# zju3dv/LoG

Hardware: AMD Instinct MI355X
Metric: Gaussians/sec fwd+bwd @1080p (higher is better)
Workload: dtype f32; 1 GPU; 30M random Gaussians (seed 0, opacity 0.999), 1920x1080, 8 orbit views/GPU, fwd+bwd; north_star / configs[3] per GPU; gaussians=30000000, width=1920, height=1080, views_per_gpu=8, streams_per_gpu=1, parallelism=single GPU, 1 view(s) in flight per GPU (HIP streams)

## Files before the change

### log_amd/csrc/blend.hip

```cpp
#include "common.hpp"
#define LR_LANDED(q0, q1, c, i)                                                                                  \
  asm volatile("" : "+v"((q0).x), "+v"((q0).y), "+v"((q0).z), "+v"((q0).w), "+v"((q1).x), "+v"((q1).y), "+v"((q1).z), \
               "+v"((q1).w), "+v"(c), "+v"(i))
#define LR_OCC_ATTR(n) __attribute__((amdgpu_waves_per_eu(n)))
#ifdef LR_OCC_BWD_ROWS_WAVES
#define LR_OCC_BWD_ROWS LR_OCC_ATTR(LR_OCC_BWD_ROWS_WAVES)
#else
#define LR_OCC_BWD_ROWS
#endif
#ifndef LR_OCC_FWD_ROWS_WAVES
#define LR_OCC_FWD_ROWS_WAVES 5
#endif
#define LR_OCC_FWD_ROWS LR_OCC_ATTR(LR_OCC_FWD_ROWS_WAVES)
#ifdef LR_OCC_BWD_WAVES
#define LR_OCC_BWD LR_OCC_ATTR(LR_OCC_BWD_WAVES)
#else
#define LR_OCC_BWD
#endif
#ifdef LR_OCC_FWD_WAVES
#define LR_OCC_FWD LR_OCC_ATTR(LR_OCC_FWD_WAVES)
#else
#define LR_OCC_FWD
#endif


LR_DEV uint32_t lr_tile_of_block(uint32_t b, uint32_t tiles, int gx, int gy, int mode,
                                 const uint32_t* __restrict__ state) {
  if (mode == 3) return b < tiles ? state[lr_order_off(tiles) + b] : 0xffffffffu;
  if (mode == 1) {
    uint32_t nper = (tiles + 7u) >> 3;
    uint32_t t = (b & 7u) * nper + (b >> 3);
    return t < tiles ? t : 0xffffffffu;
  }
  if (mode == 2) {
    uint32_t nsbx = ((uint32_t)gx + 3u) >> 2, nsby = ((uint32_t)gy + 3u) >> 2;
    uint32_t r = b >> 3, sb = (r >> 4) * 8u + (b & 7u), local = r & 15u;
    if (sb >= nsbx * nsby) return 0xffffffffu;
    uint32_t tx = (sb % nsbx) * 4u + (local & 3u), ty = (sb / nsbx) * 4u + (local >> 2);
    if (tx >= (uint32_t)gx || ty >= (uint32_t)gy) return 0xffffffffu;
    return ty * (uint32_t)gx + tx;
  }
  return b < tiles ? b : 0xffffffffu;
}
static inline __host__ __device__ uint32_t lr_blend_grid(uint32_t tiles, int gx, int gy, int mode) {
  if (mode == 1) return ((tiles + 7u) / 8u) * 8u;
  if (mode == 2) {
    uint32_t nsb = (((uint32_t)gx + 3u) >> 2) * (((uint32_t)gy + 3u) >> 2);
    return ((nsb + 7u) / 8u) * 8u * 16u;
  }
  return tiles;
}

LR_DEV bool lr_support_hits(const float4 g0, const float2 g1, float x0, float x1, float y0, float y1) {
  const float A = g0.z, B = g0.w, C = g1.x, op = g1.y;
  const float det = A * C - B * B;
  const float tau = lr_fma(__logf(255.f * op), 1.01f, 0.01f);
  if (!(op >= 1.0f / 512.0f)) return !(op < 1.0f / 512.0f);
  const float inv = 1.f / det;
  const float ex2 = 2.f * tau * C * inv, ey2 = 2.f * tau * A * inv;
  const float mag = (fabsf(A) + fabsf(B) + fabsf(C)) * (ex2 + ey2);
  const bool safe = (det > 0.f) && (ex2 >= 0.f) && (ey2 >= 0.f) && (mag * 1.0e-6f < 0.005f * tau) && (mag < 1.0e30f);
  if (!safe) return true;
  const float ex = sqrtf(ex2) + 0.01f, ey = sqrtf(ey2) + 0.01f;
  if (!((g0.x + ex >= x0) && (g0.x - ex <= x1) && (g0.y + ey >= y0) && (g0.y - ey <= y1))) return false;
  const float dx0 = (x0 - 0.01f) - g0.x, dx1 = (x1 + 0.01f) - g0.x;
  const float dy0 = (y0 - 0.01f) - g0.y, dy1 = (y1 + 0.01f) - g0.y;
  if (dx0 <= 0.f && dx1 >= 0.f && dy0 <= 0.f && dy1 >= 0.f) return true;
  const float iA = 1.f / A, iC = 1.f / C;
  float best = 3.0e38f;
#pragma unroll
  for (int e = 0; e < 2; e++) {
    const float dx = e ? dx1 : dx0;
    const float dy = fminf(dy1, fmaxf(dy0, -B * dx * iC));
    best = fminf(best, 0.5f * (A * dx * dx + C * dy * dy) + B * dx * dy);
    const float ey_ = e ? dy1 : dy0;
    const float ex_ = fminf(dx1, fmaxf(dx0, -B * ey_ * iA));
    best = fminf(best, 0.5f * (A * ex_ * ex_ + C * ey_ * ey_) + B * ex_ * ey_);
  }
  return !(best > tau);
}

LR_DEV bool lr_lazy_range(const uint32_t* sorted, uint32_t tiles, int lazy, uint32_t tile, int wave, uint32_t beg,
                          uint32_t& end, uint32_t& first, bool& clamped) {
  first = 0u;
  clamped = false;
  if (!lazy) return true;
  if (end - beg <= LR_LONG_LIST) return lazy == 1;
  const uint32_t ordered = sorted[tile] & ~63u;
  if (lazy == 1) {
    if (ordered < end - beg) { end = beg + ordered; clamped = true; }
    return true;
  }
  if (!((sorted[tiles + tile] >> wave) & 1u)) return false;
  first = ordered;
  return true;
}
template <bool EXTRAS>
LR_DEV void lr_lazy_park(const LrView& v, size_t pix, bool done, float T, float C0, float C1, float C2, int last, int wid,
                         float wmax, float* image, float* final_T, int* n_contrib, int* pid, float* pwp) {
  const size_t plane = (size_t)v.W * v.H;
  final_T[pix] = done ? -T : T;
  n_contrib[pix] = last;
  image[pix] = C0; image[plane + pix] = C1; image[2 * plane + pix] = C2;
  if (EXTRAS) { pid[pix] = wid; pwp[pix] = wmax; }
}
template <bool EXTRAS>
LR_DEV void lr_lazy_resume(const LrView& v, size_t pix, bool& done, float& T, float& C0, float& C1, float& C2, int& last,
                           int& wid, float& wmax, const float* image, const float* final_T, const int* n_contrib,
                           const int* pid, const float* pwp) {
  const size_t plane = (size_t)v.W * v.H;
  const float t = final_T[pix];
  done = t < 0.f;
  T = fabsf(t);
  last = n_contrib[pix];
  C0 = image[pix]; C1 = image[plane + pix]; C2 = image[2 * plane + pix];
  if (EXTRAS) { wid = pid[pix]; wmax = pwp[pix]; }
}

#define LR_MBUF_CHUNKS 64u
#define LR_MASK_FORM_ROWS 1u
#define LR_MASK_FORM_QUAD 2u
LR_DEV size_t lr_mask_slot(uint32_t list_begin, uint32_t tile) { return (size_t)(list_begin >> 6) + tile; }
LR_DEV uint64_t lr_mask_before(uint64_t m, int hi, int limit) {
  const int sh = hi - limit;
  return sh <= 0 ? m : (sh >= 64 ? 0ull : (m & (~0ull << sh)));
}

template <bool EXTRAS>
LR_DEV void lr_fwd_commit_chunk(uint32_t* wmx, int lane, uint32_t id_prev, float* __restrict__ pw, float4* __restrict__ zero_rows) {
  if (!EXTRAS) return;
  __builtin_amdgcn_fence(__ATOMIC_RELEASE, "wavefront");
  __builtin_amdgcn_wave_barrier();
  __builtin_amdgcn_fence(__ATOMIC_ACQUIRE, "wavefront");
  const uint32_t m = (id_prev != 0xffffffffu) ? wmx[lane] : 0u;
  if (m != 0u) atomicMax(reinterpret_cast<unsigned int*>(pw) + id_prev, m);
  if (zero_rows) {
#pragma unroll
    for (int k = 0; k < 4; k++) {
      const int e = 16 * k + (lane >> 2);
      const uint32_t me = (uint32_t)__shfl((int)m, e), ide = (uint32_t)__shfl((int)id_prev, e);
      if (me != 0u) zero_rows[4 * (size_t)ide + (lane & 3)] = float4{0.f, 0.f, 0.f, 0.f};
    }
  }
  wmx[lane] = 0u;
  __builtin_amdgcn_fence(__ATOMIC_RELEASE, "wavefront");
  __builtin_amdgcn_wave_barrier();
}

template <bool EXTRAS>
__global__ void __launch_bounds__(256) LR_OCC_FWD
lr_blend_fwd_kernel(LrView v, const float4* __restrict__ geom, const uint32_t* __restrict__ state,
                    uint32_t tiles, const uint32_t* __restrict__ plist, uint32_t capacity,
                    float* __restrict__ image, float* __restrict__ final_T, int* __restrict__ n_contrib,
                    int* __restrict__ pid, float* __restrict__ pwp, float* __restrict__ pw,
                    float4* __restrict__ zero_conic, int xcd_mode, int cull, uint32_t* __restrict__ lazy_state, int lazy,
                    uint64_t* __restrict__ masks, uint32_t* __restrict__ hdr_w) {
  if (lr_bail(state, capacity)) return;
  if (lazy == 2 && !lazy_state[LR_HDR_OPEN]) return;
  if (masks && blockIdx.x == 0 && threadIdx.x == 0) hdr_w[LR_HDR_MASKS] = LR_MASK_FORM_QUAD;
  const uint32_t tile = lr_tile_of_block(blockIdx.x, tiles, v.gx, v.gy, xcd_mode, state);
  if (tile >= tiles) return;
// ... 174 lines not shown
  const int px = qx0 + (lane & 7), py = qy0 + (lane >> 3);
  const float pxf = (float)px, pyf = (float)py;
  const float bx0 = (float)qx0, bx1 = (float)(qx0 + 7), by0 = (float)qy0, by1 = (float)(qy0 + 7);
  const bool in = (px < v.W) && (py < v.H);
  const size_t plane = (size_t)v.W * v.H;
  const size_t pix = in ? (size_t)py * v.W + px : 0;
  const float sx = 0.5f * (float)v.W, sy = 0.5f * (float)v.H;
  const float Tf = in ? final_T[pix] : 0.f;
  const int lastc = in ? n_contrib[pix] : 0;
  const float dp0 = in ? dL_dimage[pix] : 0.f;
  const float dp1 = in ? dL_dimage[plane + pix] : 0.f;
  const float dp2 = in ? dL_dimage[2 * plane + pix] : 0.f;
  const float bgdot = lr_fma(v.bg[0], dp0, lr_fma(v.bg[1], dp1, v.bg[2] * dp2));
  float T = Tf, acc0 = 0.f, acc1 = 0.f, acc2 = 0.f;
  int maxc = lastc;
#pragma unroll
  for (int off = 32; off > 0; off >>= 1) maxc = max(maxc, __shfl_xor(maxc, off));
  maxc = lr_readlane_i(maxc, 0);

  const int row = lane >> 4;
  float* const base0 = acc_rows + ((row < 3) ? 6 + row : 5);
  float* const base1 = acc_rows + ((lane == 1) ? 4 : row);
  const bool lead = (lane & 15) == 0;

  const int top = use_masks ? ((maxc + 63) & ~63) : maxc;
  const uint32_t nchunks = ((uint32_t)top + 63u) >> 6;
  auto load_id = [&](uint32_t c) -> uint32_t {
    const int pos = top - 1 - (int)(c * 64u) - lane;
    return (c < nchunks && pos >= 0 && pos < maxc) ? plist[beg + (uint32_t)pos] : 0xffffffffu;
  };
  const uint64_t* const mbase = use_masks ? masks + 4 * lr_mask_slot(beg, tile) + __builtin_amdgcn_readfirstlane(quad) : nullptr;
  auto load_mask = [&](uint32_t c) -> uint64_t {
    return (use_masks && c < nchunks) ? mbase[4 * (size_t)(((uint32_t)top >> 6) - 1u - c)] : 0ull;
  };
  uint32_t id_n = load_id(0), id_nn = load_id(1);
  uint64_t mk_n = load_mask(0), mk_nn = load_mask(1);
  float4 g0_n = {0.f, 0.f, 0.f, 0.f};
  float2 g1_n = {0.f, 0.f};
  if (!use_masks && id_n != 0xffffffffu) { g0_n = geom[LR_REC_QUADS * (size_t)id_n]; g1_n = *reinterpret_cast<const float2*>(geom + LR_REC_QUADS * (size_t)id_n + 1); }

  for (uint32_t ch = 0; ch < nchunks; ch++) {
    const int hi = top - (int)(ch * 64u);
    const uint32_t id = id_n;
    const float4 g0 = g0_n;
    const float2 g1 = g1_n;
    const uint64_t mk = mk_n;
    id_n = id_nn;
    id_nn = load_id(ch + 2);
    mk_n = mk_nn;
    mk_nn = load_mask(ch + 2);
    uint64_t todo;
    if (use_masks) {
      todo = lr_mask_before(__builtin_bitreverse64(mk), hi, maxc);
    } else {
      if (id_n != 0xffffffffu) { g0_n = geom[LR_REC_QUADS * (size_t)id_n]; g1_n = *reinterpret_cast<const float2*>(geom + LR_REC_QUADS * (size_t)id_n + 1); }
      const bool rel = (id != 0xffffffffu) && (cull ? lr_support_hits(g0, g1, bx0, bx1, by0, by1) : true);
      todo = __ballot(rel);
    }
    while (todo) {
      const int j0 = __builtin_ctzll(todo);
      todo &= todo - 1;
      const bool has1 = todo != 0;
      const int j1 = has1 ? __builtin_ctzll(todo) : j0;
      todo &= todo - 1;
      const int gid0 = lr_readlane_i((int)id, j0), gid1 = lr_readlane_i((int)id, j1);
      const float4* __restrict__ rr0 = geom + LR_REC_QUADS * (size_t)(uint32_t)gid0;
      const float4* __restrict__ rr1 = geom + LR_REC_QUADS * (size_t)(uint32_t)gid1;
      const float4 q00 = rr0[0], q01 = rr0[1], q10 = rr1[0], q11 = rr1[1];
      const float cbl0 = reinterpret_cast<const float*>(rr0)[8], cbl1 = reinterpret_cast<const float*>(rr1)[8];
      asm volatile("" : : "s"(q01.z), "s"(q01.w), "s"(cbl0), "s"(q11.z), "s"(q11.w), "s"(cbl1));
      const float op0 = q01.y, op1 = q11.y;
      const lr_f2 dx2 = lr_f2{q00.x, q10.x} - pxf, dy2 = lr_f2{q00.y, q10.y} - pyf;
      const lr_f2 hdx2 = dx2 * -0.5f, hdy2 = dy2 * -0.5f;
      const lr_f2 bdx = lr_f2{q00.w, q10.w} * dx2;
      const lr_f2 pw2 = lr_fma2(lr_f2{q00.z, q10.z} * dx2, hdx2,
                                lr_fma2(lr_f2{q01.x, q11.x} * dy2, hdy2, lr_f2{-bdx.x, -bdx.y} * dy2));
      const lr_f2 G2 = lr_exp2(pw2);
      const lr_f2 al2 = lr_f2{op0, op1} * G2;
      const float power0 = pw2.x, power1 = pw2.y, G0 = G2.x, G1 = G2.y;
      const float alpha0 = fminf(0.99f, al2.x), alpha1 = fminf(0.99f, al2.y);
      const int k0 = hi - 1 - j0, k1 = hi - 1 - j1;
      const bool hit0 = (k0 < lastc) & !(power0 > 0.f) & !(alpha0 < 1.0f / 255.0f);
      const bool hit1 = has1 & (k1 < lastc) & !(power1 > 0.f) & !(alpha1 < 1.0f / 255.0f);
      const lr_f2 alpha = {hit0 ? alpha0 : 0.f, hit1 ? alpha1 : 0.f};
      const bool any0 = __builtin_amdgcn_ballot_w64(alpha.x > 0.f) != 0, any1 = __builtin_amdgcn_ballot_w64(alpha.y > 0.f) != 0;
      if (!(any0 | any1)) continue;
      const lr_f2 G = {hit0 ? G0 : 0.f, hit1 ? G1 : 0.f};
      const lr_f2 om = 1.f - alpha;
      lr_f2 rc = {__builtin_amdgcn_rcpf(om.x), __builtin_amdgcn_rcpf(om.y)};
      rc = lr_fma2(lr_fma2(-om, rc, lr_f2{1.f, 1.f}), rc, rc);
      const float Ta = T * rc.x, Tb = Ta * rc.y;
      const lr_f2 T2 = {Ta, Tb};
      T = Tb;
      const lr_f2 w = alpha * T2;
      const lr_f2 cr = {q01.z, q11.z}, cg = {q01.w, q11.w}, cbl = {cbl0, cbl1};
      const float a0r = lr_fma(alpha.x, cr.x, om.x * acc0), a0g = lr_fma(alpha.x, cg.x, om.x * acc1),
                  a0b = lr_fma(alpha.x, cbl.x, om.x * acc2);
      lr_f2 dL_dalpha = lr_fma2(cr - lr_f2{acc0, a0r}, lr_f2{dp0, dp0},
                                lr_fma2(cg - lr_f2{acc1, a0g}, lr_f2{dp1, dp1}, (cbl - lr_f2{acc2, a0b}) * dp2));
      dL_dalpha = lr_fma2(dL_dalpha, T2, -(Tf * rc) * bgdot);
      acc0 = lr_fma(alpha.y, cr.y, om.y * a0r);
      acc1 = lr_fma(alpha.y, cg.y, om.y * a0g);
      acc2 = lr_fma(alpha.y, cbl.y, om.y * a0b);
      const lr_f2 Ar = {q00.z, q10.z}, Br = {q00.w, q10.w}, Cr = {q01.x, q11.x};
      const lr_f2 dL_dG = lr_f2{op0, op1} * dL_dalpha;
      const lr_f2 gdx = G * dx2, gdy = G * dy2;
      const lr_f2 dG_ddx = lr_fma2(-Ar, gdx, -(Br * gdy));
      const lr_f2 dG_ddy = lr_fma2(-Cr, gdy, -(Br * gdx));
      lr_f2 s2[9];
      s2[0] = w * dp0; s2[2] = w * dp1; s2[1] = w * dp2; s2[3] = G * dL_dalpha;
      s2[4] = dL_dG * dG_ddx * sx; s2[6] = dL_dG * dG_ddy * sy;
      s2[5] = -0.5f * gdx * dx2 * dL_dG; s2[7] = -gdx * dy2 * dL_dG;
      s2[8] = -0.5f * gdy * dy2 * dL_dG;
#pragma unroll
      for (int e = 0; e < 2; e++) {
        if (!(e ? any1 : any0)) continue;
        const int gid = e ? gid1 : gid0;
        float sv[9];
#pragma unroll
        for (int m = 0; m < 9; m++) sv[m] = e ? s2[m].y : s2[m].x;
        float r0, r1, r2;
        lr_reduce9(sv, r0, r1, r2);
        if (lead) atomicAdd(base0 + (size_t)gid * LOGRAST_BWD_ROW_FLOATS, r0);
        if (lead || lane == 1) atomicAdd(base1 + (size_t)gid * LOGRAST_BWD_ROW_FLOATS, lane == 1 ? r2 : r1);
      }
    }
  }
}

#define LR_RB_SLOT 3
template <int CTRL>
LR_DEV float lr_dpp_perm(float x) {
  return __int_as_float(__builtin_amdgcn_update_dpp(0, __float_as_int(x), CTRL, 0xf, 0xf, true));
}
template <int BANKS>
LR_DEV float lr_bank_select(float keep, float take) {
  return __int_as_float(__builtin_amdgcn_update_dpp(__float_as_int(keep), __float_as_int(take), 0xE4, 0xf, BANKS, false));
}
LR_DEV float lr_row_pair8(float a, float b) {
  return lr_bank_select<0xc>(a + lr_dpp_perm<0x140>(a), b + lr_dpp_perm<0x140>(b));
}
LR_DEV float lr_row_pair4(float p, float q) {
  return lr_bank_select<0xa>(p + lr_dpp_perm<0x141>(p), q + lr_dpp_perm<0x141>(q));
}
LR_DEV float lr_quad_total(float x) {
  x = x + lr_dpp_perm<0xB1>(x);
  return x + lr_dpp_perm<0x4E>(x);
}

LR_DEV void lr_atomic_add_noret(float* p, float x) {
  asm volatile("global_atomic_add_f32 %0, %1, off" : : "v"(p), "v"(x) : "memory");
}

LR_DEV uint32_t lr_take_bit(uint64_t& m) {
  const uint32_t j = min((uint32_t)(__ffsll((long long)m) - 1), 64u);
  m &= m - 1ull;
  return j;
}
LR_DEV uint64_t lr_row_mask(int row, uint64_t m0, uint64_t m1, uint64_t m2, uint64_t m3) {
  return row == 0 ? m0 : (row == 1 ? m1 : (row == 2 ? m2 : m3));
}

template <bool MASKS>
__global__ void __launch_bounds__(256) LR_OCC_BWD_ROWS
lr_blend_bwd_rows_kernel(LrView v, const float4* __restrict__ geom, const uint32_t* __restrict__ state,
                         uint32_t tiles, const uint32_t* __restrict__ plist, uint32_t capacity,
                         const float* __restrict__ final_T, const int* __restrict__ n_contrib,
                         const float* __restrict__ dL_dimage, float* __restrict__ acc_rows,
                         int xcd_mode, int cull, int block_test, const uint64_t* __restrict__ masks LR_ABLATE_PARAM) {
  __shared__ float4 lr_stage[4][65 * LR_RB_SLOT];
  if (lr_bail(state, capacity)) return;
  const uint32_t tile = lr_tile_of_block(blockIdx.x, tiles, v.gx, v.gy, xcd_mode, state);
  if (tile >= tiles) return;
  const uint32_t* offsets = state + lr_offsets_off(tiles);
  const uint32_t beg = offsets[tile];
  const int lane = threadIdx.x & 63, wq = threadIdx.x >> 6;
  constexpr bool use_masks = MASKS;
  const int row = lane >> 4, li = lane & 15;
  const int tx = tile % (uint32_t)v.gx, ty = tile / (uint32_t)v.gx;
  const int qx0 = tx * 16 + (wq & 1) * 8, qy0 = ty * 16 + (wq >> 1) * 8;
  const int px = qx0 + (row & 1) * 4 + (li & 3), py = qy0 + (row >> 1) * 4 + (li >> 2);
  const float pxf = (float)px, pyf = (float)py;
  const bool in = (px < v.W) && (py < v.H);
  const size_t plane = (size_t)v.W * v.H;
  const size_t pix = in ? (size_t)py * v.W + px : 0;
  const float sx = 0.5f * (float)v.W, sy = 0.5f * (float)v.H;
  const float Tf = in ? final_T[pix] : 0.f;
  const int lastc = in ? n_contrib[pix] : 0;
  const float dp0 = in ? dL_dimage[pix] : 0.f;
  const float dp1 = in ? dL_dimage[plane + pix] : 0.f;
  const float dp2 = in ? dL_dimage[2 * plane + pix] : 0.f;
  const float bgdot = lr_fma(v.bg[0], dp0, lr_fma(v.bg[1], dp1, v.bg[2] * dp2));
  float T = Tf, acc0 = 0.f, acc1 = 0.f, acc2 = 0.f;
  int rmax = lastc;
#pragma unroll
  for (int off = 8; off > 0; off >>= 1) rmax = max(rmax, __shfl_xor(rmax, off));
  const int rm0 = lr_readlane_i(rmax, 0), rm1 = lr_readlane_i(rmax, 16), rm2 = lr_readlane_i(rmax, 32),
            rm3 = lr_readlane_i(rmax, 48);
  const int maxc = max(max(rm0, rm1), max(rm2, rm3));
  if (maxc == 0) return;

  float* const sf = reinterpret_cast<float*>(lr_stage[wq]);
#define LR_SF(f, j) sf[(f) * 65 + (j)]
  const uint32_t sf_lds = (uint32_t)(uintptr_t)(__attribute__((address_space(3))) float*)sf;
  if (lane < 10) LR_SF(lane, 64) = lane == 9 ? __uint_as_float(0xffffffffu) : 0.f;

  const int qd = li >> 2, sel = li & 3;
  const int slot = sel == 0 ? (qd == 0 ? 6 : (qd == 1 ? 8 : (qd == 2 ? 7 : 5)))
                            : (sel == 1 ? (qd == 0 ? 0 : (qd == 1 ? 2 : (qd == 2 ? 1 : 3))) : 4);
  const bool on_a = sel < 2 || li == 2, on_b = sel < 2 || li == 10;
  float* const dst = acc_rows + slot;

  const float bx[2] = {(float)qx0, (float)(qx0 + 4)}, by[2] = {(float)qy0, (float)(qy0 + 4)};

  const int top = use_masks ? ((maxc + 63) & ~63) : maxc;
  const uint32_t nchunks = ((uint32_t)top + 63u) >> 6;
  auto load_id = [&](uint32_t c) -> uint32_t {
    const int pos = top - 1 - (int)(c * 64u) - lane;
    const bool ok = c < nchunks && pos >= 0 && pos < maxc;
    const uint32_t got = plist[beg + (ok ? (uint32_t)pos : 0u)];
    return ok ? got : 0xffffffffu;
  };
  const uint4* const mbase = use_masks ? reinterpret_cast<const uint4*>(masks + 16 * lr_mask_slot(beg, tile) +
                                                                        4 * __builtin_amdgcn_readfirstlane(wq)) : nullptr;
  struct Masks4 { uint64_t m0, m1, m2, m3; };
  auto load_masks = [&](uint32_t c) -> Masks4 {
    if (!use_masks) return Masks4{0ull, 0ull, 0ull, 0ull};
    const uint32_t cf = ((uint32_t)top >> 6) - 1u - min(c, nchunks - 1u);
    const uint4* mp = mbase + 8 * (size_t)cf;
    const uint4 lo = mp[0], hi4 = mp[1];
    return Masks4{((uint64_t)lo.y << 32) | lo.x, ((uint64_t)lo.w << 32) | lo.z,
                  ((uint64_t)hi4.y << 32) | hi4.x, ((uint64_t)hi4.w << 32) | hi4.z};
  };
  auto wanted = [&](const Masks4& m) -> bool {
    return !use_masks || (((m.m0 | m.m1 | m.m2 | m.m3) >> (63 - lane)) & 1ull) != 0ull;
  };
  auto gather = [&](uint32_t idv, bool want, float4& q0, float4& q1, float& qc) {
    const float4* rp = geom + LR_REC_QUADS * (size_t)(want ? idv : 0u);
    q0 = rp[0]; q1 = rp[1]; qc = reinterpret_cast<const float*>(rp)[8];
  };
  uint32_t id_n = load_id(0), id_nn = load_id(1);
  Masks4 mk_n = load_masks(0), mk_nn = load_masks(1);
  float4 g0_n, g1_n;
  float cb_n;
  gather(id_n, id_n != 0xffffffffu && wanted(mk_n), g0_n, g1_n, cb_n);
  LR_LANDED(g0_n, g1_n, cb_n, id_nn);

  for (uint32_t ch = 0; ch < nchunks; ch++) {
    const int hi = top - (int)(ch * 64u);
    const uint32_t id = id_n;
    const float4 g0 = g0_n, g1 = g1_n;
    const float cb = cb_n;
    const Masks4 mk = mk_n;
    id_n = id_nn;
    mk_n = mk_nn;
    gather(id_n, id_n != 0xffffffffu && wanted(mk_n), g0_n, g1_n, cb_n);
    id_nn = load_id(ch + 2);
    mk_nn = load_masks(ch + 2);
    __builtin_amdgcn_fence(__ATOMIC_RELEASE, "wavefront");
    __builtin_amdgcn_wave_barrier();
    if (id != 0xffffffffu && wanted(mk)) {
      LR_SF(0, lane) = g0.x; LR_SF(1, lane) = g0.y; LR_SF(2, lane) = g0.z; LR_SF(3, lane) = g0.w;
      LR_SF(4, lane) = g1.x; LR_SF(5, lane) = g1.y; LR_SF(6, lane) = g1.z; LR_SF(7, lane) = g1.w;
      LR_SF(8, lane) = cb; LR_SF(9, lane) = __uint_as_float(id);
    }
    __builtin_amdgcn_fence(__ATOMIC_RELEASE, "wavefront");
    __builtin_amdgcn_wave_barrier();
    __builtin_amdgcn_fence(__ATOMIC_ACQUIRE, "wavefront");
    const bool valid = id != 0xffffffffu;
    const int pos = hi - 1 - lane;
    bool r0 = valid & (pos < rm0), r1 = valid & (pos < rm1), r2 = valid & (pos < rm2), r3 = valid & (pos < rm3);
    if (cull && !use_masks) {
      const LrSupport sp = lr_support_prepare(g0.x, g0.y, g0.z, g0.w, g1.x, g1.y);
      if (block_test) {
        bool k0, k1, k2, k3;
        const lr_f2 X0 = {bx[0], bx[1]}, X1 = {bx[0] + 3.f, bx[1] + 3.f};
        lr_support_box2(sp, X0, X1, lr_f2{by[0], by[0]}, lr_f2{by[0] + 3.f, by[0] + 3.f}, k0, k1);
        lr_support_box2(sp, X0, X1, lr_f2{by[1], by[1]}, lr_f2{by[1] + 3.f, by[1] + 3.f}, k2, k3);
        r0 = r0 && k0; r1 = r1 && k1; r2 = r2 && k2; r3 = r3 && k3;
      } else {
        const bool q = lr_support_box(sp, bx[0], bx[0] + 7.f, by[0], by[0] + 7.f);
        const bool bb = sp.mode == 2;
        const bool x_lo = !bb || (sp.mx - sp.ex <= bx[0] + 3.f), x_hi = !bb || (sp.mx + sp.ex >= bx[1]);
        const bool y_lo = !bb || (sp.my - sp.ey <= by[0] + 3.f), y_hi = !bb || (sp.my + sp.ey >= by[1]);
        r0 = r0 && q && x_lo && y_lo;
        r1 = r1 && q && x_hi && y_lo;
        r2 = r2 && q && x_lo && y_hi;
        r3 = r3 && q && x_hi && y_hi;
      }
    }
    uint64_t mrow;
    if (use_masks) mrow = lr_mask_before(lr_row_mask(row, __builtin_bitreverse64(mk.m0), __builtin_bitreverse64(mk.m1),
                                                     __builtin_bitreverse64(mk.m2), __builtin_bitreverse64(mk.m3)), hi, rmax);
    else mrow = lr_row_mask(row, __ballot(r0), __ballot(r1), __ballot(r2), __ballot(r3));
    if (LR_ABLATED(4)) mrow = 0ull;
    while (__builtin_amdgcn_ballot_w64(mrow != 0ull) != 0) {
      const uint32_t ja = lr_take_bit(mrow), jb = lr_take_bit(mrow);
      float fa[10], fb[10];
      {
        const uint32_t aa = sf_lds + 4u * ja, ab = sf_lds + 4u * jb;
        asm volatile(
            "ds_read_b32 %0, %20\n ds_read_b32 %10, %21\n"
            "ds_read_b32 %1, %20 offset:260\n ds_read_b32 %11, %21 offset:260\n"
            "ds_read_b32 %2, %20 offset:520\n ds_read_b32 %12, %21 offset:520\n"
            "ds_read_b32 %3, %20 offset:780\n ds_read_b32 %13, %21 offset:780\n"
            "ds_read_b32 %4, %20 offset:1040\n ds_read_b32 %14, %21 offset:1040\n"
            "ds_read_b32 %5, %20 offset:1300\n ds_read_b32 %15, %21 offset:1300\n"
            "ds_read_b32 %6, %20 offset:1560\n ds_read_b32 %16, %21 offset:1560\n"
            "ds_read_b32 %7, %20 offset:1820\n ds_read_b32 %17, %21 offset:1820\n"
            "ds_read_b32 %8, %20 offset:2080\n ds_read_b32 %18, %21 offset:2080\n"
            "ds_read_b32 %9, %20 offset:2340\n ds_read_b32 %19, %21 offset:2340\n"
            "s_waitcnt lgkmcnt(0)"
            : "=&v"(fa[0]), "=&v"(fa[1]), "=&v"(fa[2]), "=&v"(fa[3]), "=&v"(fa[4]), "=&v"(fa[5]), "=&v"(fa[6]), "=&v"(fa[7]),
              "=&v"(fa[8]), "=&v"(fa[9]), "=&v"(fb[0]), "=&v"(fb[1]), "=&v"(fb[2]), "=&v"(fb[3]), "=&v"(fb[4]), "=&v"(fb[5]),
              "=&v"(fb[6]), "=&v"(fb[7]), "=&v"(fb[8]), "=&v"(fb[9])
            : "v"(aa), "v"(ab)
            : "memory");
      }
      const lr_f2 Ar = {fa[2], fb[2]}, Br = {fa[3], fb[3]}, Cr = {fa[4], fb[4]};
      const lr_f2 op2 = {fa[5], fb[5]};
      const lr_f2 cr = {fa[6], fb[6]}, cg = {fa[7], fb[7]}, cbl = {fa[8], fb[8]};
      const uint32_t gida = __float_as_uint(fa[9]), gidb = __float_as_uint(fb[9]);
      const lr_f2 dx2 = lr_f2{fa[0], fb[0]} - pxf, dy2 = lr_f2{fa[1], fb[1]} - pyf;
      const lr_f2 hdx2 = dx2 * -0.5f, hdy2 = dy2 * -0.5f;
      const lr_f2 bdx = Br * dx2;
      const lr_f2 pw2 = lr_fma2(Ar * dx2, hdx2, lr_fma2(Cr * dy2, hdy2, lr_f2{-bdx.x, -bdx.y} * dy2));
      const lr_f2 G2 = lr_exp2(pw2);
      const lr_f2 al2 = op2 * G2;
      const float alpha0 = fminf(0.99f, al2.x), alpha1 = fminf(0.99f, al2.y);
      const int k0 = hi - 1 - (int)ja, k1 = hi - 1 - (int)jb;
      const bool hit0 = (k0 < lastc) & !(pw2.x > 0.f) & !(alpha0 < 1.0f / 255.0f);
      const bool hit1 = (k1 < lastc) & !(pw2.y > 0.f) & !(alpha1 < 1.0f / 255.0f);
      const lr_f2 alpha = {hit0 ? alpha0 : 0.f, hit1 ? alpha1 : 0.f};
      const bool any = __builtin_amdgcn_ballot_w64((alpha.x > 0.f) | (alpha.y > 0.f)) != 0;
      if (!any) continue;
      const lr_f2 G = {hit0 ? G2.x : 0.f, hit1 ? G2.y : 0.f};
      const lr_f2 om = 1.f - alpha;
      lr_f2 rc = {__builtin_amdgcn_rcpf(om.x), __builtin_amdgcn_rcpf(om.y)};
      rc = lr_fma2(lr_fma2(-om, rc, lr_f2{1.f, 1.f}), rc, rc);
      const float Ta = T * rc.x, Tb = Ta * rc.y;
      const lr_f2 T2 = {Ta, Tb};
      T = Tb;
      const lr_f2 w = alpha * T2;
      const float a0r = lr_fma(alpha.x, cr.x, om.x * acc0), a0g = lr_fma(alpha.x, cg.x, om.x * acc1),
                  a0b = lr_fma(alpha.x, cbl.x, om.x * acc2);
      lr_f2 dL_dalpha = lr_fma2(cr - lr_f2{acc0, a0r}, lr_f2{dp0, dp0},
                                lr_fma2(cg - lr_f2{acc1, a0g}, lr_f2{dp1, dp1}, (cbl - lr_f2{acc2, a0b}) * dp2));
      dL_dalpha = lr_fma2(dL_dalpha, T2, -(Tf * rc) * bgdot);
      acc0 = lr_fma(alpha.y, cr.y, om.y * a0r);
      acc1 = lr_fma(alpha.y, cg.y, om.y * a0g);
      acc2 = lr_fma(alpha.y, cbl.y, om.y * a0b);
      const lr_f2 dL_dG = op2 * dL_dalpha;
      const lr_f2 gdx = G * dx2, gdy = G * dy2;
      const lr_f2 dG_ddx = lr_fma2(-Ar, gdx, -(Br * gdy));
      const lr_f2 dG_ddy = lr_fma2(-Cr, gdy, -(Br * gdx));
      const lr_f2 c0 = w * dp0, c1 = w * dp1, c2 = w * dp2, go = G * dL_dalpha;
      const lr_f2 mxs = dL_dG * dG_ddx * sx, mys = dL_dG * dG_ddy * sy;
      const lr_f2 kA = -0.5f * gdx * dx2 * dL_dG, kB = -gdx * dy2 * dL_dG, kC = -0.5f * gdy * dy2 * dL_dG;
      const float s1a = lr_quad_total(lr_row_pair4(lr_row_pair8(c0.x, c1.x), lr_row_pair8(c2.x, go.x)));
      const float s1b = lr_quad_total(lr_row_pair4(lr_row_pair8(c0.y, c1.y), lr_row_pair8(c2.y, go.y)));
      const float s2a = lr_quad_total(lr_row_pair4(lr_row_pair8(mxs.x, mys.x), lr_row_pair8(kA.x, kB.x)));
      const float s2b = lr_quad_total(lr_row_pair4(lr_row_pair8(mxs.y, mys.y), lr_row_pair8(kA.y, kB.y)));
      float s3 = lr_row_pair8(kC.x, kC.y);
      s3 = lr_quad_total(s3 + lr_dpp_perm<0x141>(s3));
      const float xa = sel == 0 ? s1a : (sel == 1 ? s2a : s3);
      const float xb = sel == 0 ? s1b : (sel == 1 ? s2b : s3);
      if (!LR_ABLATED(1)) {
        if (on_a && gida != 0xffffffffu) lr_atomic_add_noret(dst + (size_t)gida * LOGRAST_BWD_ROW_FLOATS, xa);
        if (on_b && gidb != 0xffffffffu) lr_atomic_add_noret(dst + (size_t)gidb * LOGRAST_BWD_ROW_FLOATS, xb);
      }
    }
  }
}

template <bool EXTRAS>
__global__ void __launch_bounds__(256) LR_OCC_FWD_ROWS
lr_blend_fwd_rows_kernel(LrView v, const float4* __restrict__ geom, const uint32_t* __restrict__ state,
                         uint32_t tiles, const uint32_t* __restrict__ plist, uint32_t capacity,
                         float* __restrict__ image, float* __restrict__ final_T, int* __restrict__ n_contrib,
                         int* __restrict__ pid, float* __restrict__ pwp, float* __restrict__ pw,
                         float4* __restrict__ zero_rows, int xcd_mode, int cull, uint32_t* __restrict__ lazy_state,
                         int lazy, uint64_t* __restrict__ masks, uint32_t* __restrict__ hdr_w, int block_test LR_ABLATE_PARAM) {
  __shared__ float4 lr_stage[4][65 * LR_RB_SLOT];
  if (lr_bail(state, capacity)) return;
  if (lazy == 2 && !lazy_state[LR_HDR_OPEN]) return;
  if (masks && blockIdx.x == 0 && threadIdx.x == 0) hdr_w[LR_HDR_MASKS] = LR_MASK_FORM_ROWS;
  const uint32_t tile = lr_tile_of_block(blockIdx.x, tiles, v.gx, v.gy, xcd_mode, state);
  if (tile >= tiles) return;
  const uint32_t* offsets = state + lr_offsets_off(tiles);
  uint32_t beg = offsets[tile];
  uint32_t end = offsets[tile + 1], first;
  bool clamped;
  const int lane = threadIdx.x & 63, wq = threadIdx.x >> 6;
  __shared__ uint64_t lr_mbuf[4][LR_MBUF_CHUNKS * 4];
  __shared__ uint32_t lr_wmax_r[4][65];
  uint32_t* const wmx = lr_wmax_r[wq];
  if (EXTRAS) { wmx[lane] = 0u; if (lane == 0) wmx[64] = 0u; }
  uint32_t id_prev = 0xffffffffu;
  uint64_t* const mslot = masks ? masks + 16 * lr_mask_slot(beg, tile) + 4 * wq : nullptr;
  uint32_t mcount = 0;
  uint32_t mfirst = 0;
  auto flush_masks = [&]() {
    __builtin_amdgcn_fence(__ATOMIC_RELEASE, "wavefront");
    __builtin_amdgcn_wave_barrier();
    __builtin_amdgcn_fence(__ATOMIC_ACQUIRE, "wavefront");
    if (!LR_ABLATED(8))
    for (uint32_t i = (uint32_t)lane; i < mcount * 4u; i += 64u)
      mslot[16 * (size_t)(mfirst + (i >> 2)) + (i & 3u)] = lr_mbuf[wq][i];
    __builtin_amdgcn_fence(__ATOMIC_RELEASE, "wavefront");
    __builtin_amdgcn_wave_barrier();
    mfirst += mcount;
    mcount = 0;
  };
  if (!lr_lazy_range(lazy_state + lr_sorted_off(tiles), tiles, lazy, tile, wq, beg, end, first, clamped)) return;
  const int row = lane >> 4, li = lane & 15;
  const int tx = tile % (uint32_t)v.gx, ty = tile / (uint32_t)v.gx;
  const int qx0 = tx * 16 + (wq & 1) * 8, qy0 = ty * 16 + (wq >> 1) * 8;
  const int px = qx0 + (row & 1) * 4 + (li & 3), py = qy0 + (row >> 1) * 4 + (li >> 2);
  const float pxf = (float)px, pyf = (float)py;
  const bool inside = (px < v.W) && (py < v.H);
  const size_t pix = inside ? (size_t)py * v.W + px : 0;
  bool done = !inside;
  float T = 1.f, C0 = 0.f, C1 = 0.f, C2 = 0.f, wmax = 0.f;
  int wid = -1, last = 0;
  if (lazy == 2) {
    if (inside) lr_lazy_resume<EXTRAS>(v, pix, done, T, C0, C1, C2, last, wid, wmax, image, final_T, n_contrib, pid, pwp);
    beg += first;
  }
  float4* const stage = lr_stage[wq];
  if (lane < LR_RB_SLOT) stage[64 * LR_RB_SLOT + lane] = float4{0.f, 0.f, 0.f, 0.f};
  if (lane == 2) stage[64 * LR_RB_SLOT + 2] = float4{0.f, __uint_as_float(0xffffffffu), 0.f, 0.f};
  const uint32_t shift16 = 16u * (uint32_t)row;
  const float bx[2] = {(float)qx0, (float)(qx0 + 4)}, by[2] = {(float)qy0, (float)(qy0 + 4)};
  const uint64_t rowbits = 0xffffull;

  const uint32_t nchunks = (end - beg + 63u) >> 6;
  if (end == beg) {
    if (inside && lazy != 2) {
      const size_t plane = (size_t)v.W * v.H;
      final_T[pix] = 1.f; n_contrib[pix] = 0;
      image[pix] = v.bg[0]; image[plane + pix] = v.bg[1]; image[2 * plane + pix] = v.bg[2];
      if (EXTRAS) { pid[pix] = -1; pwp[pix] = 0.f; }
    }
    return;
  }
  auto load_id = [&](uint32_t c) -> uint32_t {
    const uint32_t idx = beg + c * 64u + (uint32_t)lane;
    const bool ok = c < nchunks && idx < end;
    const uint32_t got = plist[ok ? idx : beg];
    return ok ? got : 0xffffffffu;
  };
  auto gather = [&](uint32_t idv, float4& q0, float4& q1, float& qc) {
    const float4* rp = geom + LR_REC_QUADS * (size_t)(idv != 0xffffffffu ? idv : 0u);
    q0 = rp[0]; q1 = rp[1]; qc = reinterpret_cast<const float*>(rp)[8];
  };
  uint32_t id_n = load_id(0), id_nn = load_id(1);
  float4 g0_n, g1_n;
  float cb_n;
  gather(id_n, g0_n, g1_n, cb_n);
  LR_LANDED(g0_n, g1_n, cb_n, id_nn);

  for (uint32_t ch = 0; ch < nchunks; ch++) {
    if (__all(done)) break;
    lr_fwd_commit_chunk<EXTRAS>(wmx, lane, id_prev, pw, zero_rows);
    const uint32_t id = id_n;
    id_prev = id;
    const float4 g0 = g0_n, g1 = g1_n;
    const float cb = cb_n;
    id_n = id_nn;
    gather(id_n, g0_n, g1_n, cb_n);
    id_nn = load_id(ch + 2);
    __builtin_amdgcn_fence(__ATOMIC_RELEASE, "wavefront");
    __builtin_amdgcn_wave_barrier();
    stage[lane * LR_RB_SLOT + 0] = g0;
    stage[lane * LR_RB_SLOT + 1] = g1;
    stage[lane * LR_RB_SLOT + 2] = float4{cb, __uint_as_float(id), 0.f, 0.f};
    __builtin_amdgcn_fence(__ATOMIC_RELEASE, "wavefront");
    __builtin_amdgcn_wave_barrier();
    __builtin_amdgcn_fence(__ATOMIC_ACQUIRE, "wavefront");
    const bool valid = id != 0xffffffffu;
    bool r0 = valid, r1 = valid, r2 = valid, r3 = valid;
    if (cull) {
      const LrSupport sp = lr_support_prepare(g0.x, g0.y, g0.z, g0.w, g1.x, g1.y);
      if (block_test) {
        bool k0, k1, k2, k3;
        const lr_f2 X0 = {bx[0], bx[1]}, X1 = {bx[0] + 3.f, bx[1] + 3.f};
        lr_support_box2(sp, X0, X1, lr_f2{by[0], by[0]}, lr_f2{by[0] + 3.f, by[0] + 3.f}, k0, k1);
        lr_support_box2(sp, X0, X1, lr_f2{by[1], by[1]}, lr_f2{by[1] + 3.f, by[1] + 3.f}, k2, k3);
        r0 = r0 && k0; r1 = r1 && k1; r2 = r2 && k2; r3 = r3 && k3;
      } else {
        const bool q = lr_support_box(sp, bx[0], bx[0] + 7.f, by[0], by[0] + 7.f);
        const bool bb = sp.mode == 2;
        const bool x_lo = !bb || (sp.mx - sp.ex <= bx[0] + 3.f), x_hi = !bb || (sp.mx + sp.ex >= bx[1]);
        const bool y_lo = !bb || (sp.my - sp.ey <= by[0] + 3.f), y_hi = !bb || (sp.my + sp.ey >= by[1]);
        r0 = r0 && q && x_lo && y_lo;
        r1 = r1 && q && x_hi && y_lo;
        r2 = r2 && q && x_lo && y_hi;
        r3 = r3 && q && x_hi && y_hi;
      }
    }
    uint64_t mrow = lr_row_mask(row, __ballot(r0), __ballot(r1), __ballot(r2), __ballot(r3));
    const int pos0 = (int)(first + ch * 64u);
    if (mslot) {
      if (mcount == 0) mfirst = (uint32_t)pos0 >> 6;
      if (li == 0 && !LR_ABLATED(16)) lr_mbuf[wq][mcount * 4u + (uint32_t)row] = mrow;
      if (++mcount == LR_MBUF_CHUNKS) flush_masks();
    }
    if (LR_ABLATED(4)) mrow = 0ull;
    while (true) {
      const uint64_t dm = __ballot(done);
      if ((uint32_t)((dm >> shift16) & rowbits) == (uint32_t)rowbits) mrow = 0ull;
      if (__builtin_amdgcn_ballot_w64(mrow != 0ull) == 0) break;
      const uint32_t ja = lr_take_bit(mrow), jb = lr_take_bit(mrow);
      const float4* sa = stage + ja * LR_RB_SLOT;
      const float4* sb = stage + jb * LR_RB_SLOT;
      const float4 a0 = sa[0], a1 = sa[1], a2 = sa[2], b0 = sb[0], b1 = sb[1], b2 = sb[2];
      const int gida = (int)__float_as_uint(a2.y), gidb = (int)__float_as_uint(b2.y);
      const float op0 = a1.y, op1 = b1.y;
      const lr_f2 dx2 = lr_f2{a0.x, b0.x} - pxf, dy2 = lr_f2{a0.y, b0.y} - pyf;
      const lr_f2 hdx2 = dx2 * -0.5f, hdy2 = dy2 * -0.5f;
      const lr_f2 bdx = lr_f2{a0.w, b0.w} * dx2;
      const lr_f2 pw2 = lr_fma2(lr_f2{a0.z, b0.z} * dx2, hdx2,
                                lr_fma2(lr_f2{a1.x, b1.x} * dy2, hdy2, lr_f2{-bdx.x, -bdx.y} * dy2));
      const lr_f2 al2 = lr_f2{op0, op1} * lr_exp2(pw2);
      const float alpha0 = fminf(0.99f, al2.x), alpha1 = fminf(0.99f, al2.y);
      const bool ok0 = !done & !(pw2.x > 0.f) & !(alpha0 < 1.0f / 255.0f);
      const float test0 = T * (1.f - alpha0);
      const bool stop0 = ok0 & (test0 < 0.0001f);
      const bool acc0 = ok0 & !stop0;
      const float w0 = acc0 ? alpha0 * T : 0.f;
      T = acc0 ? test0 : T;
      last = acc0 ? pos0 + (int)ja + 1 : last;
      done = done | stop0;
      const bool ok1 = !done & !(pw2.y > 0.f) & !(alpha1 < 1.0f / 255.0f);
      const float test1 = T * (1.f - alpha1);
      const bool stop1 = ok1 & (test1 < 0.0001f);
      const bool acc1 = ok1 & !stop1;
      const float w1 = acc1 ? alpha1 * T : 0.f;
      T = acc1 ? test1 : T;
      last = acc1 ? pos0 + (int)jb + 1 : last;
      done = done | stop1;
      const bool hit = __builtin_amdgcn_ballot_w64((w0 > 0.f) | (w1 > 0.f)) != 0;
      if (!hit) continue;
      if (acc0) { C0 = lr_fma(a1.z, w0, C0); C1 = lr_fma(a1.w, w0, C1); C2 = lr_fma(a2.x, w0, C2); }
      if (acc1) { C0 = lr_fma(b1.z, w1, C0); C1 = lr_fma(b1.w, w1, C1); C2 = lr_fma(b2.x, w1, C2); }
      if (EXTRAS) {
        if (w0 > wmax) { wmax = w0; wid = gida; }
        if (w1 > wmax) { wmax = w1; wid = gidb; }
        uint32_t ma = __float_as_uint(w0), mb = __float_as_uint(w1);
#define LR_RMAX(x, CTRL) x = max(x, (uint32_t)__builtin_amdgcn_update_dpp(0, (int)x, CTRL, 0xf, 0xf, true))
        LR_RMAX(ma, 0x140); LR_RMAX(mb, 0x140);
        LR_RMAX(ma, 0x141); LR_RMAX(mb, 0x141);
        LR_RMAX(ma, 0xB1); LR_RMAX(mb, 0xB1);
        LR_RMAX(ma, 0x4E); LR_RMAX(mb, 0x4E);
#undef LR_RMAX
        if (li == 0 && ma != 0u && !LR_ABLATED(1)) atomicMax(&wmx[ja], ma);
        if (li == 0 && mb != 0u && !LR_ABLATED(1)) atomicMax(&wmx[jb], mb);
      }
    }
  }
  if (mslot && mcount) flush_masks();
  lr_fwd_commit_chunk<EXTRAS>(wmx, lane, id_prev, pw, zero_rows);
  if (clamped && !__all(done)) {
    if (lane == 0) { atomicOr(lazy_state + lr_sorted_off(tiles) + tiles + tile, 1u << wq); atomicOr(lazy_state + LR_HDR_OPEN, 1u); }
    if (inside) lr_lazy_park<EXTRAS>(v, pix, done, T, C0, C1, C2, last, wid, wmax, image, final_T, n_contrib, pid, pwp);
    return;
  }

  if (inside) {
    const size_t plane = (size_t)v.W * v.H;
    final_T[pix] = T;
    n_contrib[pix] = last;
    image[pix] = lr_fma(T, v.bg[0], C0);
    image[plane + pix] = lr_fma(T, v.bg[1], C1);
    image[2 * plane + pix] = lr_fma(T, v.bg[2], C2);
    if (EXTRAS) { pid[pix] = wid; pwp[pix] = wmax; }
  }
}

int lr_blend_fwd_form(const LrView& v) {
  LR_KNOB(rows_knob, "LOGRAST_FWD_ROWS", 2);
  const int rows = rows_knob != 2 ? rows_knob : (v.walk_form == LOGRAST_FORM_ROWS ? 1 : 0);
  return rows ? (int)LR_MASK_FORM_ROWS : (int)LR_MASK_FORM_QUAD;
}

void lr_launch_blend_fwd(const LrView& v, const void* geom, const uint32_t* state, uint32_t tiles,
                         const uint32_t* plist, uint32_t capacity, float* image, float* final_T, int* n_contrib,
                         int* pid, float* pwp, float* pw, float* zero_conic, int big_input, int lazy, uint64_t* masks,
                         hipStream_t s) {
  uint32_t* const hdr_w = const_cast<uint32_t*>(state);
  uint32_t* const lazy_state = lazy ? const_cast<uint32_t*>(state) : nullptr;
  LR_KNOB(xcd_knob, "LOGRAST_XCD_MODE", 3);
  int xcd_mode = xcd_knob;
  static const int cull = LR_EXPERIMENT_INT("LOGRAST_CULL", 1);
  static const size_t lds_fwd = (size_t)LR_EXPERIMENT_INT("LOGRAST_BLEND_FWD_LDS_KB", 0) * 1024;
#ifdef LR_EXPERIMENTS
  static const int fwd_ablate = lr_env_int("LOGRAST_FWD_ABLATE", 0);
#endif
  const int rows = lr_blend_fwd_form(v) == (int)LR_MASK_FORM_ROWS;
  LR_KNOB(fwd_block_test, "LOGRAST_FWD_BLOCK_TEST", 1);
  if (!cull) masks = nullptr;
  uint32_t grid = lr_blend_grid(tiles, v.gx, v.gy, xcd_mode);
  if (lazy == 2) {
    xcd_mode = 3;
    grid = min(tiles, capacity / (uint32_t)LR_LONG_LIST + 1u);
  }
  const float4* g4 = reinterpret_cast<const float4*>(geom);
  float4* z4 = reinterpret_cast<float4*>(zero_conic);
  if (lazy != 2) lr_prof_begin(LRK_BLEND_FWD, s);
  if (rows) {
    if (v.extras)
      hipLaunchKernelGGL(lr_blend_fwd_rows_kernel<true>, dim3(grid), dim3(256), lds_fwd, s, v, g4, state, tiles, plist, capacity,
                         image, final_T, n_contrib, pid, pwp, pw, z4, xcd_mode, cull, lazy_state, lazy, masks, hdr_w, fwd_block_test LR_ABLATE_PASS(fwd_ablate));
    else
      hipLaunchKernelGGL(lr_blend_fwd_rows_kernel<false>, dim3(grid), dim3(256), lds_fwd, s, v, g4, state, tiles, plist, capacity,
                         image, final_T, n_contrib, pid, pwp, pw, z4, xcd_mode, cull, lazy_state, lazy, masks, hdr_w, fwd_block_test LR_ABLATE_PASS(fwd_ablate));
  } else {
    if (v.extras)
      hipLaunchKernelGGL(lr_blend_fwd_kernel<true>, dim3(grid), dim3(256), lds_fwd, s, v, g4, state, tiles, plist, capacity,
                         image, final_T, n_contrib, pid, pwp, pw, z4, xcd_mode, cull, lazy_state, lazy, masks, hdr_w);
    else
      hipLaunchKernelGGL(lr_blend_fwd_kernel<false>, dim3(grid), dim3(256), lds_fwd, s, v, g4, state, tiles, plist, capacity,
                         image, final_T, n_contrib, pid, pwp, pw, z4, xcd_mode, cull, lazy_state, lazy, masks, hdr_w);
  }
  if (lazy != 2) lr_prof_end(LRK_BLEND_FWD, s);
}

void lr_launch_blend_bwd(const LrView& v, const void* geom, const uint32_t* state, uint32_t tiles,
                         const uint32_t* plist, uint32_t capacity, const float* final_T, const int* n_contrib,
                         const float* dL_dimage, float* acc_rows, int big_input, const uint64_t* masks, hipStream_t s) {
  LR_KNOB(xcd_mode, "LOGRAST_XCD_MODE", 3);
  static const int cull = LR_EXPERIMENT_INT("LOGRAST_CULL", 1);
  static const size_t lds_bwd = (size_t)LR_EXPERIMENT_INT("LOGRAST_BLEND_BWD_LDS_KB", 0) * 1024;
  uint32_t grid = lr_blend_grid(tiles, v.gx, v.gy, xcd_mode);
  LR_KNOB(rows_knob, "LOGRAST_BWD_ROWS", 2);
  const int rows = rows_knob != 2 ? rows_knob
                   : (v.walk_form == LOGRAST_FORM_ROWS ? 1 : (v.walk_form == LOGRAST_FORM_QUADRANT ? 0 : (big_input ? 1 : 0)));
#ifdef LR_EXPERIMENTS
  static const int ablate = lr_env_int("LOGRAST_BWD_ABLATE", 0);
#endif
  LR_KNOB(block_test, "LOGRAST_BWD_BLOCK_TEST", 1);
  lr_prof_begin(LRK_BLEND_BWD, s);
  const bool use_masks = masks != nullptr && cull && v.mask_form == (rows ? (int)LR_MASK_FORM_ROWS : (int)LR_MASK_FORM_QUAD);
  const float4* g4 = reinterpret_cast<const float4*>(geom);
  if (rows && use_masks)
    hipLaunchKernelGGL(lr_blend_bwd_rows_kernel<true>, dim3(grid), dim3(256), lds_bwd, s, v, g4, state, tiles, plist, capacity,
                       final_T, n_contrib, dL_dimage, acc_rows, xcd_mode, cull, block_test, masks LR_ABLATE_PASS(ablate));
  else if (rows)
    hipLaunchKernelGGL(lr_blend_bwd_rows_kernel<false>, dim3(grid), dim3(256), lds_bwd, s, v, g4, state, tiles, plist, capacity,
                       final_T, n_contrib, dL_dimage, acc_rows, xcd_mode, cull, block_test, masks LR_ABLATE_PASS(ablate));
  else if (use_masks)
    hipLaunchKernelGGL(lr_blend_bwd_kernel<true>, dim3(grid), dim3(256), lds_bwd, s, v, g4, state, tiles, plist, capacity,
                       final_T, n_contrib, dL_dimage, acc_rows, xcd_mode, cull, masks);
  else
    hipLaunchKernelGGL(lr_blend_bwd_kernel<false>, dim3(grid), dim3(256), lds_bwd, s, v, g4, state, tiles, plist, capacity,
                       final_T, n_contrib, dL_dimage, acc_rows, xcd_mode, cull, masks);
  lr_prof_end(LRK_BLEND_BWD, s);
}
```

Baseline: 10.15 billion Gaussians/s.

## Accumulate backward-blend gradients in LDS per chunk before committing global atomics

The rows backward kernel now adds each per-Gaussian partial gradient into a per-wave LDS table with ds_add_f32, instead of issuing a global float atomic for every pixel-row pair. Once per 64-Gaussian chunk, the touched entries are compacted and flushed to global memory with one atomic per nonzero slot. The goal is fewer global atomics and less contention in acc_rows. The cost is extra LDS, wave barriers and a commit pass per chunk. The occupancy attribute also changes to 5 waves when masks and chunking are enabled and 1 otherwise.

```diff
diff --git a/log_amd/csrc/blend.hip b/log_amd/csrc/blend.hip
--- a/log_amd/csrc/blend.hip
+++ b/log_amd/csrc/blend.hip
@@ -6,7 +6,7 @@
 #ifdef LR_OCC_BWD_ROWS_WAVES
 #define LR_OCC_BWD_ROWS LR_OCC_ATTR(LR_OCC_BWD_ROWS_WAVES)
 #else
-#define LR_OCC_BWD_ROWS
+#define LR_OCC_BWD_ROWS LR_OCC_ATTR((MASKS && CHUNK) ? 5 : 1)
 #endif
 #ifndef LR_OCC_FWD_ROWS_WAVES
 #define LR_OCC_FWD_ROWS_WAVES 5
@@ -487,6 +487,39 @@
   asm volatile("global_atomic_add_f32 %0, %1, off" : : "v"(p), "v"(x) : "memory");
 }
 
+#define LR_BT_STRIDE 65
+LR_DEV void lr_lds_add_noret(uint32_t lds_addr, float x) {
+  asm volatile("ds_add_f32 %0, %1" : : "v"(lds_addr), "v"(x) : "memory");
+}
+LR_DEV uint64_t lr_readlane_u64(uint64_t x, int l) {
+  return ((uint64_t)(uint32_t)lr_readlane_i((int)(uint32_t)(x >> 32), l) << 32) | (uint32_t)lr_readlane_i((int)(uint32_t)x, l);
+}
+LR_DEV void lr_bwd_commit_chunk(float* tbl, const float* sf, uint64_t touched, int lane, float* __restrict__ acc_rows) {
+  if (touched == 0ull) return;
+  __builtin_amdgcn_fence(__ATOMIC_RELEASE, "wavefront");
+  __builtin_amdgcn_wave_barrier();
+  __builtin_amdgcn_fence(__ATOMIC_ACQUIRE, "wavefront");
+  const int cnt = __popcll(touched);
+  const int below = (int)__builtin_amdgcn_mbcnt_hi((uint32_t)(touched >> 32), __builtin_amdgcn_mbcnt_lo((uint32_t)touched, 0u));
+  const bool mine = ((touched >> lane) & 1ull) != 0ull;
+  const int cj = __builtin_amdgcn_ds_permute(4 * (mine ? below : cnt + (lane - below)), lane);
+  const int ce = lane / 9, cs = lane - 9 * ce;
+  for (int k = 0; 7 * k < cnt; k++) {
+    const int r = 7 * k + ce;
+    const bool ok = lane < 63 && r < cnt;
+    const int j = __builtin_amdgcn_ds_bpermute(4 * min(r, 63), cj);
+    const uint32_t gid = __float_as_uint(sf[9 * 65 + j]);
+    float* const cell = tbl + cs * LR_BT_STRIDE + j;
+    const float x = *cell;
+    if (ok) {
+      *cell = 0.f;
+      if (x != 0.f) lr_atomic_add_noret(acc_rows + (size_t)gid * LOGRAST_BWD_ROW_FLOATS + cs, x);
+    }
+  }
+  __builtin_amdgcn_fence(__ATOMIC_RELEASE, "wavefront");
+  __builtin_amdgcn_wave_barrier();
+}
+
 LR_DEV uint32_t lr_take_bit(uint64_t& m) {
   const uint32_t j = min((uint32_t)(__ffsll((long long)m) - 1), 64u);
   m &= m - 1ull;
@@ -496,7 +529,7 @@
   return row == 0 ? m0 : (row == 1 ? m1 : (row == 2 ? m2 : m3));
 }
 
-template <bool MASKS>
+template <bool MASKS, bool CHUNK>
 __global__ void __launch_bounds__(256) LR_OCC_BWD_ROWS
 lr_blend_bwd_rows_kernel(LrView v, const float4* __restrict__ geom, const uint32_t* __restrict__ state,
                          uint32_t tiles, const uint32_t* __restrict__ plist, uint32_t capacity,
@@ -545,6 +578,12 @@
                             : (sel == 1 ? (qd == 0 ? 0 : (qd == 1 ? 2 : (qd == 2 ? 1 : 3))) : 4);
   const bool on_a = sel < 2 || li == 2, on_b = sel < 2 || li == 10;
   float* const dst = acc_rows + slot;
+  __shared__ float lr_bsum[4][CHUNK ? 9 * LR_BT_STRIDE : 1];
+  float* const tbl = lr_bsum[wq];
+  const uint32_t tbl_lane = (uint32_t)(uintptr_t)(__attribute__((address_space(3))) float*)tbl + 4u * LR_BT_STRIDE * (uint32_t)slot;
+  if (CHUNK)
+    for (int i = lane; i < 9 * LR_BT_STRIDE; i += 64) tbl[i] = 0.f;
+  uint64_t touched = 0ull;
 
   const float bx[2] = {(float)qx0, (float)(qx0 + 4)}, by[2] = {(float)qy0, (float)(qy0 + 4)};
 
@@ -582,6 +621,7 @@
   LR_LANDED(g0_n, g1_n, cb_n, id_nn);
 
   for (uint32_t ch = 0; ch < nchunks; ch++) {
+    if (CHUNK) lr_bwd_commit_chunk(tbl, sf, touched, lane, acc_rows);
     const int hi = top - (int)(ch * 64u);
     const uint32_t id = id_n;
     const float4 g0 = g0_n, g1 = g1_n;
@@ -629,6 +669,7 @@
                                                      __builtin_bitreverse64(mk.m2), __builtin_bitreverse64(mk.m3)), hi, rmax);
     else mrow = lr_row_mask(row, __ballot(r0), __ballot(r1), __ballot(r2), __ballot(r3));
     if (LR_ABLATED(4)) mrow = 0ull;
+    if (CHUNK) touched = lr_readlane_u64(mrow, 0) | lr_readlane_u64(mrow, 16) | lr_readlane_u64(mrow, 32) | lr_readlane_u64(mrow, 48);
     while (__builtin_amdgcn_ballot_w64(mrow != 0ull) != 0) {
       const uint32_t ja = lr_take_bit(mrow), jb = lr_take_bit(mrow);
       float fa[10], fb[10];
@@ -700,12 +741,17 @@
       s3 = lr_quad_total(s3 + lr_dpp_perm<0x141>(s3));
       const float xa = sel == 0 ? s1a : (sel == 1 ? s2a : s3);
       const float xb = sel == 0 ? s1b : (sel == 1 ? s2b : s3);
-      if (!LR_ABLATED(1)) {
+      if (LR_ABLATED(1)) continue;
+      if (CHUNK) {
+        if (on_a) lr_lds_add_noret(tbl_lane + 4u * ja, xa);
+        if (on_b) lr_lds_add_noret(tbl_lane + 4u * jb, xb);
+      } else {
         if (on_a && gida != 0xffffffffu) lr_atomic_add_noret(dst + (size_t)gida * LOGRAST_BWD_ROW_FLOATS, xa);
         if (on_b && gidb != 0xffffffffu) lr_atomic_add_noret(dst + (size_t)gidb * LOGRAST_BWD_ROW_FLOATS, xb);
       }
     }
   }
+  if (CHUNK) lr_bwd_commit_chunk(tbl, sf, touched, lane, acc_rows);
 }
 
 template <bool EXTRAS>
@@ -975,15 +1021,16 @@
   static const int ablate = lr_env_int("LOGRAST_BWD_ABLATE", 0);
 #endif
   LR_KNOB(block_test, "LOGRAST_BWD_BLOCK_TEST", 1);
+  LR_KNOB(commit_chunk, "LOGRAST_BWD_COMMIT", 1);
   lr_prof_begin(LRK_BLEND_BWD, s);
   const bool use_masks = masks != nullptr && cull && v.mask_form == (rows ? (int)LR_MASK_FORM_ROWS : (int)LR_MASK_FORM_QUAD);
   const float4* g4 = reinterpret_cast<const float4*>(geom);
-  if (rows && use_masks)
-    hipLaunchKernelGGL(lr_blend_bwd_rows_kernel<true>, dim3(grid), dim3(256), lds_bwd, s, v, g4, state, tiles, plist, capacity,
+  if (rows) {
+    auto k = use_masks ? (commit_chunk ? lr_blend_bwd_rows_kernel<true, true> : lr_blend_bwd_rows_kernel<true, false>)
+                       : (commit_chunk ? lr_blend_bwd_rows_kernel<false, true> : lr_blend_bwd_rows_kernel<false, false>);
+    hipLaunchKernelGGL(k, dim3(grid), dim3(256), lds_bwd, s, v, g4, state, tiles, plist, capacity,
                        final_T, n_contrib, dL_dimage, acc_rows, xcd_mode, cull, block_test, masks LR_ABLATE_PASS(ablate));
-  else if (rows)
-    hipLaunchKernelGGL(lr_blend_bwd_rows_kernel<false>, dim3(grid), dim3(256), lds_bwd, s, v, g4, state, tiles, plist, capacity,
-                       final_T, n_contrib, dL_dimage, acc_rows, xcd_mode, cull, block_test, masks LR_ABLATE_PASS(ablate));
+  }
   else if (use_masks)
     hipLaunchKernelGGL(lr_blend_bwd_kernel<true>, dim3(grid), dim3(256), lds_bwd, s, v, g4, state, tiles, plist, capacity,
                        final_T, n_contrib, dL_dimage, acc_rows, xcd_mode, cull, masks);
```

New measurement: 9.662 billion Gaussians/s (median of 2 runs). 4.8% lower.
